# swiss-territorial-data-lab/proj-roadsurf

Hardware: AMD Instinct MI355X
Metric: tiles_per_sec_512x512x3 (higher is better)
Workload: dtype f16 hi + lo operand planes (22 significand bits, 3 MFMA products per product) / f32 accumulate; 1 GPU; Mask R-CNN R50-FPN inference, batch 16 of 512x512 3-band tiles per GPU (BASELINE configs[1]), 800x800 network input; seeded synthetic weights, saturated: 1000 proposals and 100 detections per tile; batch_per_gpu=16, lanes=2, lane_streams=independent, num_classes=2, weights=random

## Files before the change

### proj_roadsurf_amd/csrc/conv_wide1x1_split.hip

```cpp
#include "conv_tile.h"

namespace {

constexpr int PR = 32;
constexpr int KS = 8;
constexpr int SLICE = KS * PR * 128;
constexpr int LDS_BYTES = 2 * SLICE;

__device__ __forceinline__ float dot_term(float s, float v, float w, bool fused) {
  if (fused) return __builtin_fmaf(v, w, s);
  {
#pragma clang fp contract(off)
    const float m = v * w;
    return s + m;
  }
}

template <int NW, int NJ, int MODE>
__global__ __launch_bounds__(NW * 64, NW == 4 ? 2 : 1) void conv_wide1x1_split_kernel(const ConvParams p) {
  constexpr int BM = NW * NJ * 16;
  constexpr int NG = 32 / NW;
  constexpr int ST = MODE == 2 ? NJ : 4 * NJ;
  extern __shared__ __attribute__((aligned(16))) char smem[];
  const int tid = threadIdx.x, lane = tid & 63;
  const int wave = __builtin_amdgcn_readfirstlane(tid >> 6);
  const int M = conv_rows(p);
  const int ntiles = (M + BM - 1) / BM;
  const int q = blockIdx.x;
  if (q >= ntiles) return;
  const int m0 = xcd_tile(q, ntiles) * BM;
  const int rows = p.Cout * (MODE == 2 ? 4 : 1);
  const int npass = rows / PR;

  const int lrow = lane >> 3, lchk = lane & 7;
  const int rp = wave & 3, s0 = wave >> 2;
  const half_t* wsrc;
  {
    const int d = src_chunk(lchk, w_key(8 * rp + lrow, 8));
    wsrc = p.w + (long long)(rp * 16 + lrow) * p.Kpad + s0 * 32 + chunk_split(d, p.w_lo);
  }
  auto stage_piece = [&](int pass, int k) {
    const half_t* g = wsrc + (long long)((pass >> 1) * 64 + (pass & 1) * 8) * p.Kpad;
    char* base = smem + (pass & 1) * SLICE + (s0 * PR + rp * 8) * 128;
    glds16(g + k * (NW / 4) * 32, base + k * (NW / 4) * PR * 128);
  };

  const int fi = lane & 15, fq = lane >> 4, fkey = lane & 7;
  int w_off[2];
#pragma unroll
  for (int ii = 0; ii < 2; ++ii) w_off[ii] = frag_row(fi, ii, 8) * 128;
  const int ch_off = frag_off(fq, fkey, 0), cl_off = frag_off(fq, fkey, 1);

  half8 xh[KS][NJ], xl[KS][NJ];
  bool valid[NJ];
  long long opix[NJ];
  const float* wv[NJ];
  const bool full = m0 + (wave + 1) * NJ * 16 <= M;
#pragma unroll
  for (int j = 0; j < NJ; ++j) {
    const int m = m0 + (wave * NJ + j) * 16 + fi;
    valid[j] = m < M;
    const int mm = valid[j] ? m : M - 1;
    const Pix px = pix_of(mm, p.Wo, p.Ho);
    const int x = px.x, y = px.y, n = px.n;
    const half_t* xp = p.in + ((long long)(n * p.in_Hp + y + p.in_off) * p.in_Wp + x + p.in_off) * 256 + fq * 8;
#pragma unroll
    for (int s = 0; s < KS; ++s) { xh[s][j] = *(const half8*)(xp + s * 32); xl[s][j] = *(const half8*)(xp + p.in_lo + s * 32); }
    if (MODE == 2) {
      const int slot = p.dot_slot[n];
      wv[j] = p.dot_w + (long long)p.dot_cls[slot] * p.Cout;
      opix[j] = (long long)slot * (4 * p.Ho * p.Wo) + (long long)(2 * y) * (2 * p.Wo) + 2 * x;
    } else {
      wv[j] = nullptr;
      opix[j] = (long long)(n * p.out_Hp + y + p.out_pad) * p.out_Wp + x + p.out_pad;
    }
  }
  const bool has_res = MODE == 0 && p.res != nullptr;
  half8 rh[NJ], rl[NJ], qh[NJ], ql[NJ];
  auto load_res = [&](int pass, half8* h, half8* l) {
    const int c = (pass >> 1) * 64 + fq * 16 + (pass & 1) * 8;
#pragma unroll
    for (int j = 0; j < NJ; ++j) {
      const half_t* rp2 = p.res + opix[j] * p.out_Cs + c;
      h[j] = *(const half8*)rp2;
      l[j] = *(const half8*)(rp2 + p.res_lo);
    }
  };
#pragma unroll
  for (int j = 0; j < NJ; ++j) { rh[j] = half8{0, 0, 0, 0, 0, 0, 0, 0}; rl[j] = rh[j]; qh[j] = rh[j]; ql[j] = rh[j]; }
#pragma unroll
  for (int k = 0; k < NG; ++k) stage_piece(0, k);
  if (has_res) load_res(0, rh, rl);

#pragma unroll
  for (int s = 0; s < KS; ++s)
#pragma unroll
    for (int j = 0; j < NJ; ++j) asm volatile("" ::"v"(xh[s][j]), "v"(xl[s][j]));
  float sdot[NJ], gsum[NJ];
  half8 kh[MODE == 0 ? NJ : 1], kl[MODE == 0 ? NJ : 1];
#pragma unroll
  for (int j = 0; j < NJ; ++j) { sdot[j] = 0.f; gsum[j] = 0.f; }
  int pend = 0;
  auto run_pass = [&](const int pass, half8 (&ch)[NJ], half8 (&cl)[NJ], half8 (&nh)[NJ], half8 (&nl)[NJ]) __attribute__((always_inline)) {
    if (pend) asm volatile("s_waitcnt vmcnt(%0)" ::"n"(ST) : "memory");
    else asm volatile("s_waitcnt vmcnt(0)" ::: "memory");
    asm volatile("s_waitcnt lgkmcnt(0)" ::: "memory");
    __builtin_amdgcn_s_barrier();
    const bool more = pass + 1 < npass;
    if (more && has_res) load_res(pass + 1, nh, nl);
    const int crow = (pass >> 1) * 64 + fq * 16 + (pass & 1) * 8;
    const int g = MODE == 2 ? crow / p.Cout : 0, cb = crow - g * p.Cout;
    float bias[8], wsc[8];
    float dw[MODE == 2 ? NJ : 1][8];
    auto load_epi = [&]() {
#pragma unroll
      for (int ii = 0; ii < 2; ++ii) {
        const f32x4 b4 = *(const f32x4*)(p.bias + crow + ii * 4), s4 = *(const f32x4*)(p.wscale + crow + ii * 4);
#pragma unroll
        for (int r = 0; r < 4; ++r) { bias[ii * 4 + r] = b4[r]; wsc[ii * 4 + r] = s4[r]; }
      }
      if (MODE == 2) {
#pragma unroll
        for (int j = 0; j < NJ; ++j)
#pragma unroll
          for (int ii = 0; ii < 2; ++ii) {
            const f32x4 w4 = *(const f32x4*)(wv[j] + cb + ii * 4);
#pragma unroll
            for (int r = 0; r < 4; ++r) dw[j][ii * 4 + r] = w4[r];
          }
      }
    };
    __builtin_amdgcn_sched_barrier(0);
    const char* sb = smem + (pass & 1) * SLICE;
    f32x4 acc[2][NJ];
#pragma unroll
    for (int ii = 0; ii < 2; ++ii)
#pragma unroll
      for (int j = 0; j < NJ; ++j) acc[ii][j] = f32x4{0.f, 0.f, 0.f, 0.f};
    auto frag = [&](int s, int ii, int off) { return *(const half8*)(sb + s * (PR * 128) + w_off[ii] + off); };
    half8 wh[2], wl[2], nwh[2];
#pragma unroll
    for (int ii = 0; ii < 2; ++ii) { wh[ii] = frag(0, ii, ch_off); wl[ii] = frag(0, ii, cl_off); }
#pragma unroll
    for (int s = 0; s < KS; ++s) {
      if (s + 1 < KS) {
#pragma unroll
        for (int ii = 0; ii < 2; ++ii) nwh[ii] = frag(s + 1, ii, ch_off);
      }
      if (s == KS - 2) load_epi();
      if (more && 2 * s < NG) { stage_piece(pass + 1, 2 * s); stage_piece(pass + 1, 2 * s + 1); }
      __builtin_amdgcn_sched_barrier(0);
#pragma unroll
      for (int ii = 0; ii < 2; ++ii)
#pragma unroll
        for (int j = 0; j < NJ; ++j) acc[ii][j] = __builtin_amdgcn_mfma_f32_16x16x32_f16(wh[ii], xl[s][j], acc[ii][j], 0, 0, 0);
#pragma unroll
      for (int ii = 0; ii < 2; ++ii)
#pragma unroll
        for (int j = 0; j < NJ; ++j) acc[ii][j] = __builtin_amdgcn_mfma_f32_16x16x32_f16(wh[ii], xh[s][j], acc[ii][j], 0, 0, 0);
      __builtin_amdgcn_sched_barrier(0);
#pragma unroll
      for (int ii = 0; ii < 2; ++ii)
#pragma unroll
        for (int j = 0; j < NJ; ++j) acc[ii][j] = __builtin_amdgcn_mfma_f32_16x16x32_f16(wl[ii], xh[s][j], acc[ii][j], 0, 0, 0);
      __builtin_amdgcn_sched_barrier(0);
      if (s + 1 < KS) {
#pragma unroll
        for (int ii = 0; ii < 2; ++ii) { wl[ii] = frag(s + 1, ii, cl_off); wh[ii] = nwh[ii]; }
      }
    }

    if (MODE == 2) {
#pragma unroll
      for (int j = 0; j < NJ; ++j) {
        float v[8];
#pragma unroll
        for (int ii = 0; ii < 2; ++ii)
#pragma unroll
          for (int r = 0; r < 4; ++r) v[ii * 4 + r] = acc[ii][j][r] * wsc[ii * 4 + r] + bias[ii * 4 + r];
        if (p.relu) {
#pragma unroll
          for (int e = 0; e < 8; ++e) v[e] = v[e] > 0.f ? v[e] : 0.f;
        }
        float sd = sdot[j];
#pragma unroll
        for (int e = 0; e < 8; ++e) sd = dot_term(sd, v[e], dw[j][e], (pass & 1) == 0 && e < 4);
        sdot[j] = sd;
      }
      pend = 0;
      if (pass & 1) {
        const int blocks = p.Cout >> 6, k = (pass >> 1) % blocks;
#pragma unroll
        for (int j = 0; j < NJ; ++j) {
          float v0 = sdot[j];
          v0 += __shfl_xor(v0, 16);
          v0 += __shfl_xor(v0, 32);
          gsum[j] = k == 0 ? v0 : gsum[j] + v0;
          sdot[j] = 0.f;
        }
        if (k == blocks - 1) {
#pragma unroll
          for (int j = 0; j < NJ; ++j)
            if (fq == 0 && valid[j]) p.dot_out[opix[j] + (long long)(g >> 1) * (2 * p.Wo) + (g & 1)] = gsum[j];
          pend = full ? ST : 0;
        }
      }
    } else {
#pragma unroll
      for (int j = 0; j < NJ; ++j) {
        float v[8];
#pragma unroll
        for (int ii = 0; ii < 2; ++ii)
#pragma unroll
          for (int r = 0; r < 4; ++r) v[ii * 4 + r] = acc[ii][j][r] * wsc[ii * 4 + r] + bias[ii * 4 + r];
        if (has_res) {
#pragma unroll
          for (int e = 0; e < 8; ++e) v[e] += (float)ch[j][e] + (float)cl[j][e];
        }
        if (p.relu) {
#pragma unroll
          for (int e = 0; e < 8; ++e) v[e] = v[e] > 0.f ? v[e] : 0.f;
        }
        float scr = 0.f;
        half8 h, l;
#pragma unroll
        for (int e = 0; e < 8; ++e) {
          const float f = clamp_h16(v[e]);
          scr += __builtin_fabsf(f);
          const HiLo hl = split_round(f);
          h[e] = hl.h;
          l[e] = hl.l;
        }
        if (valid[j] && !(scr < 65504.f)) {
          unsigned c = 0;
#pragma unroll
          for (int e = 0; e < 8; ++e) c += rs_sat_bad(v[e]);
          rs_sat_flush(p.sat, c);
        }
        if ((pass & 1) == 0) {
          kh[j] = h; kl[j] = l;
        } else if (valid[j]) {
          half_t* op = (half_t*)p.out + opix[j] * p.out_Cs + crow - 8;
          *(half8*)op = kh[j];
          *(half8*)(op + 8) = h;
          *(half8*)(op + p.out_lo) = kl[j];
          *(half8*)(op + p.out_lo + 8) = l;
        }
      }
      pend = (pass & 1) && full ? ST : 0;
    }
  };
  for (int pass = 0; pass < npass; pass += 2) {
    run_pass(pass, rh, rl, qh, ql);
    run_pass(pass + 1, qh, ql, rh, rl);
  }
}

template <int NW, int NJ>
int launch_px(const ConvParams& p, hipStream_t stream) {
  const long long nblk = cdiv(p.M, NW * NJ * 16);
  RS_CHECK(nblk > 0 && nblk < (1ll << 31), RS_ERR_ARG, "conv_wide1x1_split: bad grid %lld", nblk);
  const void* k = p.mode == 2 ? (const void*)conv_wide1x1_split_kernel<NW, NJ, 2> : (const void*)conv_wide1x1_split_kernel<NW, NJ, 0>;
  static bool attr[2] = {false, false};
  const int ai = p.mode == 2 ? 1 : 0;
  if (!attr[ai]) {
    RS_HIP(hipFuncSetAttribute(k, hipFuncAttributeMaxDynamicSharedMemorySize, LDS_BYTES));
    attr[ai] = true;
  }
  ConvParams pc = p;
  void* args[] = {&pc};
  RS_HIP(hipLaunchKernel(k, dim3((unsigned)nblk), dim3(NW * 64), args, LDS_BYTES, stream));
  return RS_OK;
}

}

bool conv_wide1x1_split_ok(const ConvParams& p) {
  const int rows = p.Cout * (p.mode != 0 ? 4 : 1);
  return p.split && p.KH == 1 && p.KW == 1 && p.stride == 1 && p.Cin == 256 && p.in_Cs == 256 && p.Kpad >= 256 && !p.in2 && !p.up && !p.out_f32 &&
         !p.koff && !p.head_w && p.nseg == 0 && !p.down && !p.res32 && !p.mask && p.out_stride <= 1 && rows > 0 && rows % 64 == 0 &&
         (p.mode == 0 || (p.mode == 2 && p.Cout == 256)) &&
         p.Kpad % 8 == 0 && p.in_lo % 8 == 0 && p.w_lo % 8 == 0 &&
         (p.mode != 0 || (p.out_Cs % 8 == 0 && p.out_Cs >= rows && p.out_lo % 8 == 0 && p.res_lo % 8 == 0));
}

int launch_conv_wide1x1_split(const ConvParams& p, hipStream_t stream, int tile_px) {
  RS_CHECK(conv_wide1x1_split_ok(p), RS_ERR_UNSUPPORTED, "conv_wide1x1_split: takes split-operand 1x1 / stride 1 / Cin 256 layers with rows %% 64 == 0 (mode 0, or mode 2 with Cout 256)");
  RS_CHECK(p.M > 0 && p.in && p.w && p.bias && p.wscale && (!p.m_count || p.m_mul > 0), RS_ERR_ARG, "conv_wide1x1_split: null argument");
  if (p.mode == 2) RS_CHECK(p.dot_w && p.dot_cls && p.dot_slot && p.dot_out, RS_ERR_ARG, "conv_wide1x1_split: the fused mask predictor needs its pointers");
  else RS_CHECK(p.out, RS_ERR_ARG, "conv_wide1x1_split: null output");
  switch (tile_px) {
    case 64: return launch_px<4, 1>(p, stream);
    case 128: return launch_px<4, 2>(p, stream);
    case 256: return launch_px<8, 2>(p, stream);
    default: rs_set_error("conv_wide1x1_split: tile of %d pixels (64, 128 or 256)", tile_px); return RS_ERR_ARG;
  }
}
```

Before: 962.1 tiles/s.

## Fuse FPN top-down upsample add into split 1x1 conv; stage bias and predictor rows in LDS

```diff
diff --git a/proj_roadsurf_amd/csrc/conv_wide1x1_split.hip b/proj_roadsurf_amd/csrc/conv_wide1x1_split.hip
--- a/proj_roadsurf_amd/csrc/conv_wide1x1_split.hip
+++ b/proj_roadsurf_amd/csrc/conv_wide1x1_split.hip
@@ -6,6 +6,8 @@
 constexpr int KS = 8;
 constexpr int SLICE = KS * PR * 128;
 constexpr int LDS_BYTES = 2 * SLICE;
+constexpr int ROWS_MAX = 2048;
+constexpr int DOT_LDS_CLASSES = 4;
 
 __device__ __forceinline__ float dot_term(float s, float v, float w, bool fused) {
   if (fused) return __builtin_fmaf(v, w, s);
@@ -16,8 +18,12 @@
   }
 }
 
-template <int NW, int NJ, int MODE>
+constexpr int vmcnt_only(int n) { return (n & 15) | ((n >> 4) << 14) | (7 << 4) | (15 << 8); }
+
+template <int NW, int NJ, int MODE, bool UP, bool DL>
 __global__ __launch_bounds__(NW * 64, NW == 4 ? 2 : 1) void conv_wide1x1_split_kernel(const ConvParams p) {
+  static_assert(!UP || MODE == 0, "the top-down addend belongs to the plain layer");
+  static_assert(!DL || MODE == 2, "DL: the predictor's rows in LDS");
   constexpr int BM = NW * NJ * 16;
   constexpr int NG = 32 / NW;
   constexpr int ST = MODE == 2 ? NJ : 4 * NJ;
@@ -32,6 +38,10 @@
   const int rows = p.Cout * (MODE == 2 ? 4 : 1);
   const int npass = rows / PR;
 
+  float* const lbias = (float*)(smem + LDS_BYTES);
+  float* const lwsc = lbias + rows;
+  float* const ldot = lwsc + rows;
+
   const int lrow = lane >> 3, lchk = lane & 7;
   const int rp = wave & 3, s0 = wave >> 2;
   const half_t* wsrc;
@@ -53,8 +63,9 @@
 
   half8 xh[KS][NJ], xl[KS][NJ];
   bool valid[NJ];
-  long long opix[NJ];
-  const float* wv[NJ];
+  std::conditional_t<UP, int, long long> opix[NJ];
+  int wv[NJ];
+  int upix[UP ? NJ : 1];
   const bool full = m0 + (wave + 1) * NJ * 16 <= M;
 #pragma unroll
   for (int j = 0; j < NJ; ++j) {
@@ -68,22 +79,23 @@
     for (int s = 0; s < KS; ++s) { xh[s][j] = *(const half8*)(xp + s * 32); xl[s][j] = *(const half8*)(xp + p.in_lo + s * 32); }
     if (MODE == 2) {
       const int slot = p.dot_slot[n];
-      wv[j] = p.dot_w + (long long)p.dot_cls[slot] * p.Cout;
+      wv[j] = p.dot_cls[slot] * p.Cout;
       opix[j] = (long long)slot * (4 * p.Ho * p.Wo) + (long long)(2 * y) * (2 * p.Wo) + 2 * x;
     } else {
-      wv[j] = nullptr;
-      opix[j] = (long long)(n * p.out_Hp + y + p.out_pad) * p.out_Wp + x + p.out_pad;
+      wv[j] = 0;
+      opix[j] = (std::conditional_t<UP, int, long long>)(n * p.out_Hp + y + p.out_pad) * p.out_Wp + x + p.out_pad;
     }
-  }
-  const bool has_res = MODE == 0 && p.res != nullptr;
+    if (UP) upix[j] = (n * p.up_Hp + (y >> 1) + p.up_pad) * p.up_Wp + (x >> 1) + p.up_pad;
+  }
+  const bool has_res = MODE == 0 && (UP || p.res != nullptr);
   half8 rh[NJ], rl[NJ], qh[NJ], ql[NJ];
   auto load_res = [&](int pass, half8* h, half8* l) {
     const int c = (pass >> 1) * 64 + fq * 16 + (pass & 1) * 8;
 #pragma unroll
     for (int j = 0; j < NJ; ++j) {
-      const half_t* rp2 = p.res + opix[j] * p.out_Cs + c;
+      const half_t* rp2 = UP ? p.up + (long long)upix[j] * p.up_Cs + c : p.res + opix[j] * p.out_Cs + c;
       h[j] = *(const half8*)rp2;
-      l[j] = *(const half8*)(rp2 + p.res_lo);
+      l[j] = *(const half8*)(rp2 + (UP ? p.up_lo : p.res_lo));
     }
   };
 #pragma unroll
@@ -92,6 +104,12 @@
   for (int k = 0; k < NG; ++k) stage_piece(0, k);
   if (has_res) load_res(0, rh, rl);
 
+#pragma unroll
+  for (int i = 0; i < ROWS_MAX / 4 / (NW * 64); ++i) {
+    const int e = tid + i * NW * 64;
+    if (e < rows / 4) { ((f32x4*)lbias)[e] = ((const f32x4*)p.bias)[e]; ((f32x4*)lwsc)[e] = ((const f32x4*)p.wscale)[e]; }
+  }
+  if (DL && tid < p.dot_k * 64) ((f32x4*)ldot)[tid] = ((const f32x4*)p.dot_w)[tid];
 #pragma unroll
   for (int s = 0; s < KS; ++s)
 #pragma unroll
@@ -101,11 +119,25 @@
 #pragma unroll
   for (int j = 0; j < NJ; ++j) { sdot[j] = 0.f; gsum[j] = 0.f; }
   int pend = 0;
-  auto run_pass = [&](const int pass, half8 (&ch)[NJ], half8 (&cl)[NJ], half8 (&nh)[NJ], half8 (&nl)[NJ]) __attribute__((always_inline)) {
-    if (pend) asm volatile("s_waitcnt vmcnt(%0)" ::"n"(ST) : "memory");
-    else asm volatile("s_waitcnt vmcnt(0)" ::: "memory");
+  half8 oh[MODE == 0 ? NJ : 1], ol[MODE == 0 ? NJ : 1];
+  auto store_block = [&](const int pass0) {
+    const int c = (pass0 >> 1) * 64 + fq * 16;
+#pragma unroll
+    for (int j = 0; j < NJ; ++j)
+      if (valid[j]) {
+        half_t* op = (half_t*)p.out + (long long)opix[j] * p.out_Cs + c;
+        *(half8*)op = kh[j];
+        *(half8*)(op + 8) = oh[j];
+        *(half8*)(op + p.out_lo) = kl[j];
+        *(half8*)(op + p.out_lo + 8) = ol[j];
+      }
+  };
+  auto run_pass = [&](const int pass, const bool odd, half8 (&ch)[NJ], half8 (&cl)[NJ], half8 (&nh)[NJ], half8 (&nl)[NJ]) __attribute__((always_inline)) {
+    if (MODE == 2 && pend) __builtin_amdgcn_s_waitcnt(vmcnt_only(ST));
+    else __builtin_amdgcn_s_waitcnt(vmcnt_only(0));
     asm volatile("s_waitcnt lgkmcnt(0)" ::: "memory");
     __builtin_amdgcn_s_barrier();
+    if (MODE == 0 && !odd && pass > 0) store_block(pass - 2);
     const bool more = pass + 1 < npass;
     if (more && has_res) load_res(pass + 1, nh, nl);
     const int crow = (pass >> 1) * 64 + fq * 16 + (pass & 1) * 8;
@@ -115,7 +147,7 @@
     auto load_epi = [&]() {
 #pragma unroll
       for (int ii = 0; ii < 2; ++ii) {
-        const f32x4 b4 = *(const f32x4*)(p.bias + crow + ii * 4), s4 = *(const f32x4*)(p.wscale + crow + ii * 4);
+        const f32x4 b4 = *(const f32x4*)(lbias + crow + ii * 4), s4 = *(const f32x4*)(lwsc + crow + ii * 4);
 #pragma unroll
         for (int r = 0; r < 4; ++r) { bias[ii * 4 + r] = b4[r]; wsc[ii * 4 + r] = s4[r]; }
       }
@@ -124,7 +156,7 @@
         for (int j = 0; j < NJ; ++j)
 #pragma unroll
           for (int ii = 0; ii < 2; ++ii) {
-            const f32x4 w4 = *(const f32x4*)(wv[j] + cb + ii * 4);
+            const f32x4 w4 = *(const f32x4*)((DL ? ldot : p.dot_w) + wv[j] + cb + ii * 4);
 #pragma unroll
             for (int r = 0; r < 4; ++r) dw[j][ii * 4 + r] = w4[r];
           }
@@ -147,7 +179,7 @@
 #pragma unroll
         for (int ii = 0; ii < 2; ++ii) nwh[ii] = frag(s + 1, ii, ch_off);
       }
-      if (s == KS - 2) load_epi();
+      if (s == KS - 1) load_epi();
       if (more && 2 * s < NG) { stage_piece(pass + 1, 2 * s); stage_piece(pass + 1, 2 * s + 1); }
       __builtin_amdgcn_sched_barrier(0);
 #pragma unroll
@@ -237,39 +269,36 @@
           for (int e = 0; e < 8; ++e) c += rs_sat_bad(v[e]);
           rs_sat_flush(p.sat, c);
         }
-        if ((pass & 1) == 0) {
-          kh[j] = h; kl[j] = l;
-        } else if (valid[j]) {
-          half_t* op = (half_t*)p.out + opix[j] * p.out_Cs + crow - 8;
-          *(half8*)op = kh[j];
-          *(half8*)(op + 8) = h;
-          *(half8*)(op + p.out_lo) = kl[j];
-          *(half8*)(op + p.out_lo + 8) = l;
-        }
-      }
-      pend = (pass & 1) && full ? ST : 0;
+        if (!odd) { kh[j] = h; kl[j] = l; }
+        else { oh[j] = h; ol[j] = l; }
+      }
     }
   };
   for (int pass = 0; pass < npass; pass += 2) {
-    run_pass(pass, rh, rl, qh, ql);
-    run_pass(pass + 1, qh, ql, rh, rl);
-  }
+    run_pass(pass, false, rh, rl, qh, ql);
+    run_pass(pass + 1, true, qh, ql, rh, rl);
+  }
+  if (MODE == 0) store_block(npass - 2);
 }
 
 template <int NW, int NJ>
 int launch_px(const ConvParams& p, hipStream_t stream) {
   const long long nblk = cdiv(p.M, NW * NJ * 16);
   RS_CHECK(nblk > 0 && nblk < (1ll << 31), RS_ERR_ARG, "conv_wide1x1_split: bad grid %lld", nblk);
-  const void* k = p.mode == 2 ? (const void*)conv_wide1x1_split_kernel<NW, NJ, 2> : (const void*)conv_wide1x1_split_kernel<NW, NJ, 0>;
-  static bool attr[2] = {false, false};
-  const int ai = p.mode == 2 ? 1 : 0;
+  const int rows = p.Cout * (p.mode == 2 ? 4 : 1);
+  const bool dl = p.mode == 2 && p.dot_k <= DOT_LDS_CLASSES;
+  const void* k = p.mode == 2 ? (dl ? (const void*)conv_wide1x1_split_kernel<NW, NJ, 2, false, true> : (const void*)conv_wide1x1_split_kernel<NW, NJ, 2, false, false>)
+                  : (p.up ? (const void*)conv_wide1x1_split_kernel<NW, NJ, 0, true, false> : (const void*)conv_wide1x1_split_kernel<NW, NJ, 0, false, false>);
+  static bool attr[4] = {false, false, false, false};
+  const int ai = p.mode == 2 ? (dl ? 3 : 1) : (p.up ? 2 : 0);
   if (!attr[ai]) {
-    RS_HIP(hipFuncSetAttribute(k, hipFuncAttributeMaxDynamicSharedMemorySize, LDS_BYTES));
+    RS_HIP(hipFuncSetAttribute(k, hipFuncAttributeMaxDynamicSharedMemorySize, LDS_BYTES + 8 * ROWS_MAX));
     attr[ai] = true;
   }
+  const int lds = LDS_BYTES + 8 * rows + (dl ? p.dot_k * 1024 : 0);
   ConvParams pc = p;
   void* args[] = {&pc};
-  RS_HIP(hipLaunchKernel(k, dim3((unsigned)nblk), dim3(NW * 64), args, LDS_BYTES, stream));
+  RS_HIP(hipLaunchKernel(k, dim3((unsigned)nblk), dim3(NW * 64), args, lds, stream));
   return RS_OK;
 }
 
@@ -277,11 +306,14 @@
 
 bool conv_wide1x1_split_ok(const ConvParams& p) {
   const int rows = p.Cout * (p.mode != 0 ? 4 : 1);
-  return p.split && p.KH == 1 && p.KW == 1 && p.stride == 1 && p.Cin == 256 && p.in_Cs == 256 && p.Kpad >= 256 && !p.in2 && !p.up && !p.out_f32 &&
-         !p.koff && !p.head_w && p.nseg == 0 && !p.down && !p.res32 && !p.mask && p.out_stride <= 1 && rows > 0 && rows % 64 == 0 &&
+  return p.split && p.KH == 1 && p.KW == 1 && p.stride == 1 && p.Cin == 256 && p.in_Cs == 256 && p.Kpad >= 256 && !p.in2 && !(p.up && (p.res || p.mode != 0)) && !p.out_f32 &&
+         !p.koff && !p.head_w && p.nseg == 0 && !p.down && !p.res32 && !p.mask && p.out_stride <= 1 && rows > 0 && rows % 64 == 0 && rows <= ROWS_MAX &&
          (p.mode == 0 || (p.mode == 2 && p.Cout == 256)) &&
          p.Kpad % 8 == 0 && p.in_lo % 8 == 0 && p.w_lo % 8 == 0 &&
-         (p.mode != 0 || (p.out_Cs % 8 == 0 && p.out_Cs >= rows && p.out_lo % 8 == 0 && p.res_lo % 8 == 0));
+         (p.mode != 0 || (p.out_Cs % 8 == 0 && p.out_Cs >= rows && p.out_lo % 8 == 0 && p.res_lo % 8 == 0 &&
+                           (!p.up || (p.up_Cs % 8 == 0 && p.up_Cs >= rows && p.up_lo % 8 == 0 && p.Ho > 0 && p.Wo > 0 &&
+                                      (long long)cdiv(p.M, p.Ho * p.Wo) * p.out_Hp * p.out_Wp < (1ll << 31) &&
+                                      (long long)cdiv(p.M, p.Ho * p.Wo) * p.up_Hp * p.up_Wp < (1ll << 31)))));
 }
 
 int launch_conv_wide1x1_split(const ConvParams& p, hipStream_t stream, int tile_px) {
```

Measured after the change: 965.1 tiles/s, median of 6. About the same (+0.3%).
